# Kotomiya07/kuzushiji-vision

Hardware: AMD Instinct MI355X
Metric: line-images/sec (train) (higher is better)
Workload: dtype bf16; 1 GPU; TrOCR train step: ViT-B/16 (12L/768/12h/3072) on 64x640 crops (S_e=161) + RoBERTa decoder 6L/256/4h/768, V=4300 one-char vocab, labels [B,128], dropout 0.1, clip 1.0, RAdamScheduleFree; BASELINE.json configs[1]; per_gpu_batch=256, global_batch=256, parallelism=dp1

## Files before the change

include/kzv.h:

```cpp
#ifndef KZV_H
#define KZV_H
#include <stddef.h>
#include <stdint.h>

#ifdef __cplusplus
extern "C" {
#endif

#define KZV_OK 0
#define KZV_E_ARG (-1)
#define KZV_E_HIP (-2)
#define KZV_E_STATE (-3)

const char* kzv_last_error(void);
int kzv_version(void);

typedef struct kzv_config {
    int32_t image_h, image_w, patch_h, patch_w, channels;
    int32_t enc_hidden, enc_layers, enc_heads, enc_ffn;
    int32_t dec_hidden, dec_layers, dec_heads, dec_ffn;
    int32_t vocab, max_pos, type_vocab, pad_id;
    float enc_hidden_dropout, enc_attn_dropout, dec_hidden_dropout, dec_attn_dropout;
    float ln_eps;
} kzv_config;
// ... 89 lines not shown
    const void* B; int64_t ldb;
    void* C; int64_t ldc;
    const float* bias;
    const float* resid; int64_t ldr;
    void* aux; int64_t ldaux;
    int32_t M, N, K, n_valid;
    float drop_p; uint32_t drop_key;
} kzv_gemm_nt_args;
int kzv_gemm_nt(const kzv_gemm_nt_args* a, int epilogue, void* stream);
int kzv_set_rows_max_m(int n);
int kzv_set_nt_schedule(int n);
int kzv_set_nt_half_epilogues(int mask);
int kzv_set_nt_half_stagger(int us);
int kzv_set_tn_schedule(int n);
typedef struct kzv_gemm_rows_ln_args {
    const void* A; int64_t lda;
    const void* B; int64_t ldb;
    void* C; int64_t ldc;
    const float* bias;
    void* aux; int64_t ldaux;
    int32_t M, N, K, n_valid;
    const float* ln_a; const float* ln_a_gamma; const float* ln_a_beta;
    const float* ln_r; const float* ln_r_gamma; const float* ln_r_beta;
    float eps;
} kzv_gemm_rows_ln_args;
int kzv_gemm_rows_ln(const kzv_gemm_rows_ln_args* a, int epilogue, void* stream);

typedef struct kzv_gemm_nt_fp8_args {
    const void* A; int64_t lda;
    const void* B; int64_t ldb;
    const float* a_scale;
    const float* b_scale;
    void* C; int64_t ldc;
    const float* bias;
    const float* resid; int64_t ldr;
    void* aux; int64_t ldaux;
    void* c8; int64_t ldc8;
    const float* c8_qscale; float* c8_amax;
    int32_t M, N, K, n_valid;
    float drop_p; uint32_t drop_key;
    const float* c8_rowq;
} kzv_gemm_nt_fp8_args;
int kzv_gemm_nt_fp8(const kzv_gemm_nt_fp8_args* a, int epilogue, void* stream);
int kzv_quant_rows_fp8(const float* x, int64_t rows, int64_t cols, void* q, float* scale, void* stream);
int kzv_layernorm_fwd_fp8(const float* x, const float* gamma, const float* beta, void* y_bf16, void* y_fp8, float* y_scale,
                          float* stats, int rows, int H, float eps, void* stream);
int kzv_set_fp8(kzv_model* m, int mode);
int kzv_get_fp8(const kzv_model* m);
int kzv_fp8_act_scales(const kzv_model* m, float* d_out, void* stream);

typedef struct kzv_gemm_tn_args {
    const void* P; int64_t ldp;
    const void* Q; int64_t ldq;
    float* OUT; int64_t ldo;
    int32_t Mtok, N, K, n_store;
    float* dbias;
} kzv_gemm_tn_args;
int kzv_gemm_tn(const kzv_gemm_tn_args* a, void* stream);

int kzv_gemm_dgrad_wgrad(const kzv_gemm_nt_args* nt, int epilogue, const kzv_gemm_tn_args* tn, void* stream);
int kzv_set_pair(int on);

int kzv_gemm_nt_f32(const kzv_gemm_nt_args* a, int epilogue, void* stream);
int kzv_gemm_tn_f32(const kzv_gemm_tn_args* a, void* stream);

int kzv_layernorm_fwd(const float* x, const float* gamma, const float* beta, void* y_bf16, float* y_f32,
                      float* stats , int rows, int H, float eps, void* stream);
int kzv_layernorm_bwd(const void* dy, int dy_is_f32, const float* x, const float* stats, const float* gamma,
                      float* dx, int accumulate_dx, float* dgamma, float* dbeta, int rows, int H, void* stream);

typedef struct kzv_attn_args {
    const void* Q; const void* K; const void* V;
    void* O;
    float* LSE;
    const void* dO; void* dQ; void* dK; void* dV;
    int64_t ldq, ldk, ldv, ldo;
    const int64_t* ids; int64_t ld_ids; int32_t pad_id;
    int32_t B, heads, Sq, Sk, mode;
    float drop_p; uint32_t drop_key;
    int32_t head_dim;
} kzv_attn_args;
int kzv_attn_fwd(const kzv_attn_args* a, void* stream);
int kzv_attn_bwd(const kzv_attn_args* a, void* stream);
#define KZV_ATTN_MFMA64 1
#define KZV_ATTN_MFMA96 2
#define KZV_ATTN_VALU 3
int kzv_attn_impl(const kzv_attn_args* a, int bwd);

int kzv_attn_stream_fwd(const kzv_attn_args* a, void* stream);
int kzv_attn_stream_bwd(const kzv_attn_args* a, void* stream);
#define KZV_ATTN_STREAM64 4
#define KZV_ATTN_STREAM96 5
int kzv_attn_impl_ex(const kzv_attn_args* a, int bwd, unsigned flags);

int kzv_ocr_set_precision(int fp32);
int kzv_ocr_nchw_to_nhwc(const float* x, void* out_bf16, int N, int C, int H, int W, void* stream);
int kzv_ocr_im2col(const void* x_bf16, void* cols_bf16, int N, int H, int W, int C, int KH, int KW, int stride, int pad, int Kp, void* stream);
int kzv_ocr_col2im(const float* dcols, float* dx, int N, int H, int W, int C, int KH, int KW, int stride, int pad, int Kp, int accumulate, void* stream);
int kzv_ocr_conv_weight(const float* w, void* wp_bf16, void* wpT_bf16, int Cout, int Cin, int KH, int KW, int Kp, void* stream);
int kzv_ocr_conv_wgrad_unpack(const float* gp, float* g, int Cout, int Cin, int KH, int KW, int Kp, void* stream);
int kzv_ocr_conv_weight_multi(int n, const float* const* w, void* const* wp_bf16, void* const* wpT_bf16, const int32_t* geom, void* stream);
int kzv_ocr_conv_wgrad_unpack_multi(int n, const float* const* gp, float* const* g, const int32_t* geom, void* stream);
int64_t kzv_ocr_bn_scratch_floats(int64_t M, int C);
int kzv_ocr_bn_fwd(const float* y, int64_t M, int C, const float* gamma, const float* beta, float* run_mean, float* run_var, float* mean,
                   float* rstd, const void* resid_bf16, void* out_bf16, int relu, int train, float eps, float momentum, float* d_scratch, void* stream);
int kzv_ocr_bn_bwd(const float* da, const void* a_bf16, const float* y, int64_t M, int C, const float* mean, const float* rstd, const float* gamma,
                   float* dz, float* dgamma, float* dbeta, void* dy_bf16, int relu, int train, float* d_scratch, void* stream);
int kzv_ocr_maxpool_fwd(const void* x_bf16, void* out_bf16, unsigned char* idx, int N, int H, int W, int C, void* stream);
int kzv_ocr_maxpool_bwd(const float* dout, const unsigned char* idx, float* dx, int N, int H, int W, int C, void* stream);
int kzv_ocr_avgpool_fwd(const void* x_bf16, float* feat_f32, void* feat_bf16, int N, int HW, int C, void* stream);
int kzv_ocr_avgpool_bwd(const float* dfeat, float* dx, int N, int HW, int C, void* stream);
int kzv_ocr_lstm_cell_fwd(const float* gates, const float* b_hh, float* h_f32, void* h_bf16, int64_t ldh, int B, int H, void* stream);
int kzv_ocr_lstm_cell_bwd(const float* gates, const float* b_hh, const float* dh, int64_t lddh, void* dgates_bf16, int B, int H, void* stream);
int kzv_ocr_log_softmax(const float* x, float* lp, int rows, int C, void* stream);
int kzv_ocr_ctc(const float* lp, const int64_t* targets, int64_t ld_targets, const int64_t* input_lengths, const int64_t* target_lengths, int T,
                int B, int C, int blank, int zero_infinity, int max_target_len, float* d_scratch, float* d_nll, const float* d_gscale,
                float* d_dlogits, void* stream);
int kzv_ocr_smooth_l1_boxes(const float* pred, int max_boxes, const float* gt, int gt_boxes, const int32_t* counts, int B, float* d_loss,
                            float* d_dpred, void* stream);
int kzv_ocr_adam(float* p, const float* g, float* m, float* v, int64_t n, float lr, float beta1, float beta2, float eps, int step, void* stream);
int kzv_ocr_adam_dev(float* p, const float* g, float* m, float* v, int64_t n, float lr, float beta1, float beta2, float eps, const float* d_bc,
                     void* stream);
int kzv_ocr_cast_bf16(const float* x, void* out_bf16, int64_t n, void* stream);
int kzv_ocr_cast_transpose(const float* x, void* out_bf16, int rows, int cols, void* stream);

int kzv_prof_enable(int on, int capacity);
int kzv_prof_select(unsigned kind_mask);
int kzv_prof_collect(int kind, double* total_ms, double* total_flops, int64_t* launches);
int kzv_prof_sample(int stride);
int64_t kzv_prof_seen(int kind);
uint32_t kzv_drop_key(uint64_t seed, uint32_t site);

#define KZV_SITE_ENC_EMB 1u
#define KZV_SITE_ENC_LAYER(i, k) (16u + 4u * (uint32_t)(i) + (uint32_t)(k))
#define KZV_SITE_DEC_EMB 1000u
#define KZV_SITE_DEC_LAYER(i, k) (1016u + 8u * (uint32_t)(i) + (uint32_t)(k))

int kzv_debug_dropout_mask(uint32_t key, float p, int64_t rows, int64_t cols, int64_t ld_index, float* d_out, void* stream);
int kzv_debug_attn_dropout_mask(uint32_t key, float p, int64_t pairs, int32_t Sq, int32_t Sk, float* d_out, void* stream);

int kzv_set_cu_reserve(int n);
int kzv_get_cu_reserve(void);

typedef struct {
    int64_t src_off;
    int64_t tmp_off;
    int64_t hb_off, hk_off;
    int64_t vb_off, vk_off;
    int32_t in_h, in_w, new_h, new_w, paste_x, paste_y, hk_size, vk_size;
} kzv_line_desc;
int kzv_lanczos_coeffs(int in_size, int out_size, int32_t* bounds, int32_t* kk, int* ksize);
int kzv_preprocess_lines(const uint8_t* rgb, const kzv_line_desc* desc, const int32_t* coef, int n, int target_h, int target_w,
                         int64_t max_tmp_pixels, const float* lut256, uint8_t* tmp, float* out, void* stream);

#ifdef __cplusplus
}
#endif
#endif
```

kuzushiji-vision_amd/csrc/attention.hip:

```cpp
#define KZV_GLDS_NT
#include "attention_common.h"

namespace {


struct AttnP {
    const bf16_t* Q; const bf16_t* K; const bf16_t* V; bf16_t* O; float* LSE;
    const bf16_t* dO; bf16_t* dQ; bf16_t* dK; bf16_t* dV;
    const void* zero16;
    int64_t ldq, ldk, ldv, ldo;
    const int64_t* ids; int64_t ld_ids; int pad_id;
    int B, heads, Sq, Sk;
    float scale; unsigned thr16; float inv_keep; unsigned key;
};

template <int SP, int NW>
__device__ __forceinline__ void stage_image(char* img, const bf16_t* src, int64_t ld, int nvalid, const void* zero16,
                                            int w, int lane) {
    const int r8 = lane >> 3;
    for (int pc = w; pc < SP / 8; pc += NW) {
        const int row = pc * 8 + r8;
        const int chunk = (lane & 7) ^ swz<64>(row);
        const void* s = row < nvalid ? (const void*)(src + (int64_t)row * ld + chunk * 8) : zero16;
        glds16(s, img + pc * 1024);
    }
}

template <int MODE, int NKT, bool EXACT>
__global__ __launch_bounds__(256, NKT <= 12 ? 3 : 2) void attn_fwd_kernel(const AttnP p) {
    constexpr int NKP = (NKT + 1) / 2;
    constexpr int SPK = NKT * 16, SPV = NKP * 32;
    constexpr int QI = (NKT + 3) / 4;
    extern __shared__ __attribute__((aligned(16))) char smem[];
    char* Ks = smem; char* Vs = smem + SPK * 128;
    int* kvalid = (int*)(smem + (SPK + SPV) * 128);
    const int tid = threadIdx.x, lane = tid & 63, w = tid >> 6, g = lane >> 4, l15 = lane & 15;
    const int b = blockIdx.x / p.heads, h = blockIdx.x - b * p.heads;
#ifdef KZV_STAMPS
    unsigned long long* stp = (p.dQ && (blockIdx.x % 257) == 0 && tid == 0) ? (unsigned long long*)p.dQ + (blockIdx.x / 257) * 8 : nullptr;
    int stk = 0;
#define KZV_ASTAMP() do { if (stp) stp[stk++] = __builtin_amdgcn_s_memrealtime(); } while (0)
#else
#define KZV_ASTAMP() do {} while (0)
#endif
    KZV_ASTAMP();
    stage_image<SPK, 4>(Ks, p.K + (int64_t)b * p.Sk * p.ldk + h * 64, p.ldk, p.Sk, p.zero16, w, lane);
    stage_image<SPV, 4>(Vs, p.V + (int64_t)b * p.Sk * p.ldv + h * 64, p.ldv, p.Sk, p.zero16, w, lane);
    if (MODE == 1)
        for (int i = tid; i < SPK; i += 256) kvalid[i] = i < p.Sk && p.ids[(int64_t)b * p.ld_ids + i] != p.pad_id;
    const int nkt = EXACT ? NKT : (p.Sk + 15) >> 4, nqt = (p.Sq + 15) >> 4;
    bf16x8 qf[QI][2];
#pragma unroll
    for (int it = 0; it < QI; ++it) {
        const int qc = min((w + 4 * it) * 16 + l15, p.Sq - 1);
        const bf16_t* qrow = p.Q + ((int64_t)b * p.Sq + qc) * p.ldq + h * 64 + 8 * g;
        qf[it][0] = *(const bf16x8*)qrow; qf[it][1] = *(const bf16x8*)(qrow + 32);
    }
    const unsigned kA = l15 * 128 + ((g ^ (l15 & 7)) << 4), kB = l15 * 128 + (((4 + g) ^ (l15 & 7)) << 4);
    unsigned vT[4];
    {
        const int row = 4 * g + (l15 >> 2), hb = (l15 >> 1) & 1;
#pragma unroll
        for (int dt = 0; dt < 4; ++dt) vT[dt] = row * 128 + ((((dt * 2 + hb) ^ (row & 7))) << 4) + (l15 & 1) * 8;
    }
    const AttDropLane dl = att_drop_lane(l15 & 3, true);
    const unsigned thrm1x2 = att_thrm1x2(p.thr16);
    const unsigned nQ4 = KZV_ATT_N4(p.Sq), nK4 = KZV_ATT_N4(p.Sk);
    asm volatile("s_waitcnt vmcnt(0)" ::: "memory");
    __syncthreads();
    KZV_ASTAMP();

    const float sc = p.scale * LOG2E;
#pragma unroll
    for (int it = 0; it < QI; ++it) {
        const int qt = w + 4 * it;
        if (qt >= nqt) break;
        const int q = qt * 16 + l15;
        const bf16x8 q0 = qf[it][0], q1 = qf[it][1];
        const int nk = MODE == 1 ? min(nkt, qt + 1) : nkt;
        f32x4 s[NKT];
        float mx = -INFINITY;
#pragma unroll
        for (int kt = 0; kt < NKT; ++kt) {
            s[kt] = (f32x4){0.f, 0.f, 0.f, 0.f};
            if (EXACT || kt < nk) {
                s[kt] = __builtin_amdgcn_mfma_f32_16x16x32_bf16(*(const bf16x8*)(Ks + kA + kt * 2048), q0, s[kt], 0, 0, 0);
                s[kt] = __builtin_amdgcn_mfma_f32_16x16x32_bf16(*(const bf16x8*)(Ks + kB + kt * 2048), q1, s[kt], 0, 0, 0);
                if (MODE == 1 || (EXACT ? kt == NKT - 1 : kt >= nkt - 1)) {
#pragma unroll
                    for (int r = 0; r < 4; ++r) {
                        const int key = kt * 16 + 4 * g + r;
                        const bool ok = MODE == 0 ? key < p.Sk : (kvalid[key] && key <= q);
                        s[kt][r] = ok ? s[kt][r] : -INFINITY;
                    }
                }
                mx = fmax3(mx, fmax3(s[kt][0], s[kt][1], s[kt][2]), s[kt][3]);
            }
        }
        mx = fmaxf(mx, __shfl_xor(mx, 16, 64));
        mx = fmaxf(mx, __shfl_xor(mx, 32, 64));
        const bool dead = mx == -INFINITY;
        const float mref = dead ? 0.f : mx * sc;
        float sum = 0.f;
        unsigned pw[NKP * 4];
        const unsigned xw0 = att_block_word(b * p.heads + h, nQ4, (unsigned)q >> 2, nK4, g, p.key);
#pragma unroll
        for (int kt = 0; kt < NKP * 2; ++kt) {
            if (kt < NKT && (EXACT || kt < nk)) {
                att_fwd_tile(s[kt], sc, mref, sum, p.thr16, dl, xw0 + (unsigned)kt * (4u * KZV_ATT_GOLD), thrm1x2, pw + kt * 2);
            } else {
                pw[kt * 2] = 0u; pw[kt * 2 + 1] = 0u;
            }
        }
        sum += __shfl_xor(sum, 16, 64);
        sum += __shfl_xor(sum, 32, 64);
        if (p.LSE && g == 0 && q < p.Sq)
            p.LSE[((int64_t)b * p.heads + h) * p.Sq + q] = dead ? INFINITY : (mx * sc + log2f(sum)) * (1.f / LOG2E);
        f32x4 o[4];
#pragma unroll
        for (int dt = 0; dt < 4; ++dt) o[dt] = (f32x4){0.f, 0.f, 0.f, 0.f};
#pragma unroll
        for (int kp = 0; kp < NKP; ++kp) {
            if (EXACT || 2 * kp < nk) {
                const bf16x8 pf = words8(pw[kp * 4], pw[kp * 4 + 1], pw[kp * 4 + 2], pw[kp * 4 + 3]);
#pragma unroll
                for (int dt = 0; dt < 4; ++dt) {
                    const bf16x8 vf = cat8(lds_tr16(Vs + vT[dt] + kp * 4096), lds_tr16(Vs + vT[dt] + kp * 4096 + 2048));
                    o[dt] = __builtin_amdgcn_mfma_f32_16x16x32_bf16(vf, pf, o[dt], 0, 0, 0);
                }
            }
        }
        const float onorm = dead ? 0.f : p.inv_keep / sum;
        if (q < p.Sq) {
            bf16_t* orow = p.O + ((int64_t)b * p.Sq + q) * p.ldo + h * 64 + 4 * g;
#pragma unroll
            for (int dt = 0; dt < 4; ++dt)
                store_bf4(orow + dt * 16, o[dt], onorm);
        }
        KZV_ASTAMP();
    }
}

constexpr int SLAB = 32 * 128;
constexpr bool bwd_ds(int MODE, int NKT, int NW, bool EXACT) { return NW == 4 && (EXACT || (MODE == 1 && NKT <= 8)); }
constexpr int bwd_lds_bytes(int NKT, int MODE, bool DS) {
    return ((NKT + 1) / 2 * 32) * 128 + NKT * 16 * 128 + 4 * SLAB + ((NKT + 1) / 2 * 32) * 64 + (MODE == 1 ? 3 : 2) * ((NKT + 1) / 2 * 32) * 4 + (DS ? SLAB : 0);
}
static_assert(bwd_lds_bytes(11, 0, true) <= 80 * 1024 && bwd_lds_bytes(12, 0, false) <= 80 * 1024 && bwd_lds_bytes(8, 1, true) <= 80 * 1024,
              "attention backward (<= 192 tokens) must fit two workgroups per CU");

template <int NW>
__device__ __forceinline__ void stage_slabs(char* qs, char* os, const bf16_t* Qb, const bf16_t* dOb, unsigned ldq, unsigned ldo,
                                            int row0, int nvalid, int w, int lane, char* oo = nullptr, const bf16_t* Ob = nullptr) {
    const int npc = oo ? 12 : 8;
    for (int pc = w; pc < npc; pc += NW) {
        const int pq = pc & 3;
        const int row = pq * 8 + (lane >> 3);
        const unsigned chunk = (lane & 7) ^ swz<64>(row);
        const unsigned r = (unsigned)min(row0 + row, nvalid - 1);
        if (pc < 4) glds16_asm_soff_m0(Qb, (r * ldq + chunk * 8) * 2, qs + pq * 1024);
        else if (pc < 8) glds16_asm_soff_m0(dOb, (r * ldo + chunk * 8) * 2, os + pq * 1024);
        else glds16_asm_soff_m0(Ob, (r * ldo + chunk * 8) * 2, oo + pq * 1024);
    }
}
__device__ __forceinline__ void slab_delta(const char* os, const char* oo, float* dlt_slab, float keep_p, int w, int lane) {
    const int row = w * 8 + (lane >> 3);
    const unsigned off = img_off<64>(row, lane & 7);
    const bf16x8 a = *(const bf16x8*)(os + off), e = *(const bf16x8*)(oo + off);
    float d = dot8(a, e);
    d += __shfl_xor(d, 1, 64);
    d += __shfl_xor(d, 2, 64);
    d += __shfl_xor(d, 4, 64);
    if ((lane & 7) == 0) dlt_slab[row] = d * keep_p;
}
template <int SP, int NW>
__device__ __forceinline__ void stage_image_asm(char* img, const bf16_t* src, int64_t ld, int nvalid, const void* zero16,
                                                int w, int lane) {
    const int r8 = lane >> 3;
    for (int pc = w; pc < SP / 8; pc += NW) {
        const int row = pc * 8 + r8;
        const int chunk = (lane & 7) ^ swz<64>(row);
        glds16_asm_m0(row < nvalid ? (const void*)(src + (int64_t)row * ld + chunk * 8) : zero16, img + pc * 1024);
    }
}

#ifdef KZV_STAMPS
__device__ unsigned long long kzv_bwd_stamps[128];
#define KZV_BSTAMP() do { if (blockIdx.x == 771 && threadIdx.x == 0 && bsk < 128) kzv_bwd_stamps[bsk++] = __builtin_amdgcn_s_memrealtime(); } while (0)
#else
#define KZV_BSTAMP() do {} while (0)
#endif
template <int MODE, int NKT, int NW, bool EXACT>
__global__ __launch_bounds__(NW * 64, 2) void attn_bwd_kernel(const AttnP p) {
    [[maybe_unused]] int bsk = 0;
    KZV_BSTAMP();
    constexpr int NKP = (NKT + 1) / 2, SP = NKP * 32;
    constexpr int NT = NW * 64, TPW = (NKT + NW - 1) / NW, TB = 8 / NW;
    static_assert(TPW <= 3, "dK/dV accumulators of more than 3 key tiles per wave do not fit the register file");
    extern __shared__ __attribute__((aligned(16))) char smem[];
    char* Ks = smem; char* Vs = Ks + SP * 128;
    char* Qring = Vs + NKT * 16 * 128; char* Oring = Qring + 2 * SLAB;
    char* dST = Oring + 2 * SLAB;
    constexpr bool DS = bwd_ds(MODE, NKT, NW, EXACT);
    float* lse = (float*)(dST + SP * 64);
    float* dlt = lse + SP;
    char* Oo = (char*)(dlt + SP);
    int* kvalid = (int*)(Oo + (DS ? SLAB : 0));
    const int tid = threadIdx.x, lane = tid & 63, w = tid >> 6, g = lane >> 4, l15 = lane & 15;
    const int b = blockIdx.x / p.heads, h = blockIdx.x - b * p.heads;
    const bf16_t* Qb = p.Q + (int64_t)b * p.Sq * p.ldq + h * 64;
    const bf16_t* dOb = p.dO + (int64_t)b * p.Sq * p.ldo + h * 64;
    const bf16_t* Ob = p.O + (int64_t)b * p.Sq * p.ldo + h * 64;
    const float keep_p = 1.f / p.inv_keep;
  if constexpr (DS) {
    float lv = INFINITY;
    if (tid < SP && tid < p.Sq) lv = p.LSE[((int64_t)b * p.heads + h) * p.Sq + tid] * LOG2E;
    stage_slabs<NW>(Qring, Oring, Qb, dOb, (unsigned)p.ldq, (unsigned)p.ldo, 0, p.Sq, w, lane, Oo, Ob);
    stage_image_asm<SP, NW>(Ks, p.K + (int64_t)b * p.Sk * p.ldk + h * 64, p.ldk, p.Sk, p.zero16, w, lane);
    stage_image_asm<NKT * 16, NW>(Vs, p.V + (int64_t)b * p.Sk * p.ldv + h * 64, p.ldv, p.Sk, p.zero16, w, lane);
    KZV_BSTAMP();
    if (tid < SP) lse[tid] = lv;
    for (int row = tid; row < SP; row += NT) if (row >= 32) dlt[row] = 0.f;
    KZV_BSTAMP();
  } else {
    constexpr int DR = (SP + NT / 4 - 1) / (NT / 4);
    bf16x8 ov[DR][2], dv8[DR][2];
    float lv[DR];
#pragma unroll
    for (int i = 0; i < DR; ++i) {
        const int row = min((tid >> 2) + i * (NT / 4), p.Sq - 1);
        const bf16_t* orow = p.O + ((int64_t)b * p.Sq + row) * p.ldo + h * 64 + (tid & 3) * 16;
        const bf16_t* drow = dOb + (int64_t)row * p.ldo + (tid & 3) * 16;
        ov[i][0] = *(const bf16x8*)orow; ov[i][1] = *(const bf16x8*)(orow + 8);
        dv8[i][0] = *(const bf16x8*)drow; dv8[i][1] = *(const bf16x8*)(drow + 8);
        lv[i] = p.LSE[((int64_t)b * p.heads + h) * p.Sq + row];
    }
    stage_image_asm<SP, NW>(Ks, p.K + (int64_t)b * p.Sk * p.ldk + h * 64, p.ldk, p.Sk, p.zero16, w, lane);
    stage_image_asm<NKT * 16, NW>(Vs, p.V + (int64_t)b * p.Sk * p.ldv + h * 64, p.ldv, p.Sk, p.zero16, w, lane);
    stage_slabs<NW>(Qring, Oring, Qb, dOb, (unsigned)p.ldq, (unsigned)p.ldo, 0, p.Sq, w, lane);
    KZV_BSTAMP();
#pragma unroll
    for (int i = 0; i < DR; ++i) {
        const int row = (tid >> 2) + i * (NT / 4);
        float d = 0.f;
#pragma unroll
        for (int c = 0; c < 2; ++c) d = dot8(ov[i][c], dv8[i][c], d);
        att_row_stats(d, lv[i], keep_p, row, SP, p.Sq, tid, lse, dlt);
    }
    KZV_BSTAMP();
  }
    if (MODE == 1)
        for (int row = tid; row < SP; row += NT) kvalid[row] = row < p.Sk && p.ids[(int64_t)b * p.ld_ids + row] != p.pad_id;
    for (int i = tid; i < SP * 64 / 16; i += NT) ((uint4*)dST)[i] = make_uint4(0, 0, 0, 0);
    asm volatile("s_waitcnt vmcnt(0)" ::: "memory");
    if constexpr (DS) slab_delta(Oring, Oo, dlt, keep_p, w, lane);
    __syncthreads();
    KZV_BSTAMP();

    const int nkt = EXACT ? NKT : (p.Sk + 15) >> 4, nqb = (p.Sq + 31) >> 5;
    const float sc = p.scale * LOG2E;
    f32x4 dk[TPW][4], dv[TPW][4];
#pragma unroll
    for (int a = 0; a < TPW; ++a)
#pragma unroll
        for (int d = 0; d < 4; ++d) { dk[a][d] = (f32x4){0.f, 0.f, 0.f, 0.f}; dv[a][d] = (f32x4){0.f, 0.f, 0.f, 0.f}; }
    const unsigned rA = img_off<64>(l15, g), rB = img_off<64>(l15, 4 + g);
    unsigned tT[4];
    {
        const int row = 4 * g + (l15 >> 2), hb = (l15 >> 1) & 1;
#pragma unroll
        for (int dt = 0; dt < 4; ++dt) tT[dt] = row * 128 + ((((dt * 2 + hb) ^ (row & 7))) << 4) + (l15 & 1) * 8;
    }
    const AttDropLane dl = att_drop_lane(l15 & 3, false);
    const int thr_s = att_thr_s(p.thr16);
    const unsigned nQ4 = KZV_ATT_N4(p.Sq), nK4 = KZV_ATT_N4(p.Sk);
    unsigned xslab = att_block_word(b * p.heads + h, nQ4, g, nK4, l15 >> 2, p.key);
    const unsigned xstep_t2 = 4u * nK4 * KZV_ATT_GOLD;

    for (int qb = 0; qb < nqb; ++qb) {
        const char* Qs = Qring + (qb & 1) * SLAB;
        const char* Os = Oring + (qb & 1) * SLAB;
        bf16x8 Qr[2][2], Or[2][2];
#pragma unroll
        for (int t2 = 0; t2 < 2; ++t2) {
            Qr[t2][0] = *(const bf16x8*)(Qs + rA + t2 * 2048); Qr[t2][1] = *(const bf16x8*)(Qs + rB + t2 * 2048);
            Or[t2][0] = *(const bf16x8*)(Os + rA + t2 * 2048); Or[t2][1] = *(const bf16x8*)(Os + rB + t2 * 2048);
        }
        if (qb + 1 < nqb)
            stage_slabs<NW>(Qring + ((qb + 1) & 1) * SLAB, Oring + ((qb + 1) & 1) * SLAB, Qb, dOb, (unsigned)p.ldq, (unsigned)p.ldo, (qb + 1) * 32, p.Sq, w, lane,
                            DS ? Oo : nullptr, Ob);
        KZV_BSTAMP();
#pragma unroll
        for (int a = 0; a < TPW; ++a) {
            const int kt = w + NW * a;
            if (kt >= nkt) continue;
            const int key = kt * 16 + l15;
            char* dsrow = dST + key * 64;
            const int dsz = (key >> 1) & 7;
            if (MODE == 1 && kt * 16 > qb * 32 + 31) {
#pragma unroll
                for (int t2 = 0; t2 < 2; ++t2) *(uint2*)(dsrow + (((t2 * 4 + g) ^ dsz) << 3)) = make_uint2(0u, 0u);
                continue;
            }
            const bf16x8 k0 = *(const bf16x8*)(Ks + rA + kt * 2048), k1 = *(const bf16x8*)(Ks + rB + kt * 2048);
            const bf16x8 v0 = *(const bf16x8*)(Vs + rA + kt * 2048), v1 = *(const bf16x8*)(Vs + rB + kt * 2048);
            const bool kok = MODE == 1 ? kvalid[key] != 0 : key < p.Sk;
            const float sinit = kok ? 0.f : -INFINITY;
            unsigned pdw[4], dsw[4];
#pragma unroll
            for (int t2 = 0; t2 < 2; ++t2) {
                const f32x4 lq4 = *(const f32x4*)(lse + qb * 32 + t2 * 16 + 4 * g), dq4 = *(const f32x4*)(dlt + qb * 32 + t2 * 16 + 4 * g);
                f32x4 S = (f32x4){sinit, sinit, sinit, sinit}, dP = (f32x4){0.f, 0.f, 0.f, 0.f};
                S = __builtin_amdgcn_mfma_f32_16x16x32_bf16(Qr[t2][0], k0, S, 0, 0, 0);
                S = __builtin_amdgcn_mfma_f32_16x16x32_bf16(Qr[t2][1], k1, S, 0, 0, 0);
                dP = __builtin_amdgcn_mfma_f32_16x16x32_bf16(Or[t2][0], v0, dP, 0, 0, 0);
                dP = __builtin_amdgcn_mfma_f32_16x16x32_bf16(Or[t2][1], v1, dP, 0, 0, 0);
                unsigned u01 = 0, u23 = 0;
                if (p.thr16)
                    att_drop_u(dl, att_mix(xslab + (unsigned)t2 * xstep_t2 + (unsigned)kt * (4u * KZV_ATT_GOLD)), &u01, &u23);
                float pm[4], ds[4];
#pragma unroll
                for (int r = 0; r < 4; ++r)
                    att_bwd_elem<MODE == 1>(r, S[r], dP[r], sc, lq4[r], dq4[r], key <= qb * 32 + t2 * 16 + 4 * g + r, u01, u23, thr_s, pm[r], ds[r]);
                pdw[t2 * 2] = pack_bf2(pm[0], pm[1]); pdw[t2 * 2 + 1] = pack_bf2(pm[2], pm[3]);
                dsw[t2 * 2] = pack_bf2(ds[0], ds[1]); dsw[t2 * 2 + 1] = pack_bf2(ds[2], ds[3]);
                *(uint2*)(dsrow + (((t2 * 4 + g) ^ dsz) << 3)) = make_uint2(dsw[t2 * 2], dsw[t2 * 2 + 1]);
            }
            const bf16x8 pf = words8(pdw[0], pdw[1], pdw[2], pdw[3]), df = words8(dsw[0], dsw[1], dsw[2], dsw[3]);
#pragma unroll
            for (int dt = 0; dt < 4; ++dt) {
                const bf16x8 dOt = cat8(lds_tr16(Os + tT[dt]), lds_tr16(Os + tT[dt] + 2048));
                const bf16x8 Qt = cat8(lds_tr16(Qs + tT[dt]), lds_tr16(Qs + tT[dt] + 2048));
                dv[a][dt] = __builtin_amdgcn_mfma_f32_16x16x32_bf16(dOt, pf, dv[a][dt], 0, 0, 0);
                dk[a][dt] = __builtin_amdgcn_mfma_f32_16x16x32_bf16(Qt, df, dk[a][dt], 0, 0, 0);
            }
            KZV_BSTAMP();
        }
        KZV_BSTAMP();
        __syncthreads();
        KZV_BSTAMP();
        {
            const int t2 = w / (NW / 2), dt0 = (w % (NW / 2)) * TB;
            const int q = qb * 32 + t2 * 16 + l15;
            f32x4 acc[TB];
#pragma unroll
            for (int u = 0; u < TB; ++u) acc[u] = (f32x4){0.f, 0.f, 0.f, 0.f};
            const int krow = 8 * g + (l15 >> 2);
            const unsigned dA = krow * 64 + (((t2 * 4 + (l15 & 3)) ^ ((krow >> 1) & 7)) << 3);
            const unsigned dB = (krow + 4) * 64 + (((t2 * 4 + (l15 & 3)) ^ (((krow + 4) >> 1) & 7)) << 3);
            unsigned kT[TB][2];
#pragma unroll
            for (int u = 0; u < TB; ++u) {
                const int row = 8 * g + (l15 >> 2), chunk = (dt0 + u) * 2 + ((l15 >> 1) & 1);
                kT[u][0] = row * 128 + ((chunk ^ (row & 7)) << 4) + (l15 & 1) * 8;
                kT[u][1] = (row + 4) * 128 + ((chunk ^ ((row + 4) & 7)) << 4) + (l15 & 1) * 8;
            }
            const int nks = EXACT ? NKP : (nkt + 1) >> 1;
#pragma unroll
            for (int ks = 0; ks < NKP; ++ks) {
                if (EXACT || ks < nks) {
                    const bf16x8 dsf = cat8(lds_tr16(dST + dA + ks * 2048), lds_tr16(dST + dB + ks * 2048));
#pragma unroll
                    for (int u = 0; u < TB; ++u) {
                        const bf16x8 kf = cat8(lds_tr16(Ks + kT[u][0] + ks * 4096), lds_tr16(Ks + kT[u][1] + ks * 4096));
                        acc[u] = __builtin_amdgcn_mfma_f32_16x16x32_bf16(kf, dsf, acc[u], 0, 0, 0);
                    }
                }
            }
            KZV_BSTAMP();
            asm volatile("s_waitcnt vmcnt(0)" ::: "memory");
            if constexpr (DS)
                if (qb + 1 < nqb) slab_delta(Oring + ((qb + 1) & 1) * SLAB, Oo, dlt + (qb + 1) * 32, keep_p, w, lane);
            if (q < p.Sq) {
                const float osc = p.scale * p.inv_keep;
                bf16_t* row = p.dQ + ((int64_t)b * p.Sq + q) * p.ldq + h * 64 + 4 * g;
#pragma unroll
                for (int u = 0; u < TB; ++u) {
                    const int dt = dt0 + u;
                    *(uint2*)(row + dt * 16) = make_uint2(pack_bf2(acc[u][0] * osc, acc[u][1] * osc), pack_bf2(acc[u][2] * osc, acc[u][3] * osc));
                }
            }
        }
        xslab += 2u * xstep_t2;
        KZV_BSTAMP();
        __syncthreads();
        KZV_BSTAMP();
    }
    const float ksc = p.scale * p.inv_keep;
#pragma unroll
    for (int a = 0; a < TPW; ++a) {
        const int key = (w + NW * a) * 16 + l15;
        if (w + NW * a >= nkt || key >= p.Sk) continue;
        bf16_t* krow = p.dK + ((int64_t)b * p.Sk + key) * p.ldk + h * 64 + 4 * g;
        bf16_t* vrow = p.dV + ((int64_t)b * p.Sk + key) * p.ldv + h * 64 + 4 * g;
#pragma unroll
        for (int dt = 0; dt < 4; ++dt) {
            store_bf4(krow + dt * 16, dk[a][dt], ksc);
            store_bf4(vrow + dt * 16, dv[a][dt], p.inv_keep);
        }
    }
}

}

#ifdef KZV_STAMPS
extern "C" int kzv_debug_bwd_stamps(unsigned long long* host128) {
    return hipMemcpyFromSymbol(host128, HIP_SYMBOL(kzv_bwd_stamps), 128 * sizeof(unsigned long long)) == hipSuccess ? 0 : 1;
}
#endif

template <int MODE, int NKT, bool EXACT>
static void launch_fwd(const AttnP& p, int blocks, hipStream_t s) {
    constexpr int lds = (NKT * 16 + (NKT + 1) / 2 * 32) * 128 + NKT * 16 * 4;
    static bool attr = false;
    if (!attr) { (void)hipFuncSetAttribute((const void*)attn_fwd_kernel<MODE, NKT, EXACT>, hipFuncAttributeMaxDynamicSharedMemorySize, lds); attr = true; }
    hipLaunchKernelGGL((attn_fwd_kernel<MODE, NKT, EXACT>), dim3(blocks), dim3(256), lds, s, p);
}
template <int MODE, int NKT, int NW, bool EXACT>
static void launch_bwd(const AttnP& p, int blocks, hipStream_t s) {
    constexpr int lds = bwd_lds_bytes(NKT, MODE, bwd_ds(MODE, NKT, NW, EXACT));
    static bool attr = false;
    if (!attr) { (void)hipFuncSetAttribute((const void*)attn_bwd_kernel<MODE, NKT, NW, EXACT>, hipFuncAttributeMaxDynamicSharedMemorySize, lds); attr = true; }
    hipLaunchKernelGGL((attn_bwd_kernel<MODE, NKT, NW, EXACT>), dim3(blocks), dim3(NW * 64), lds, s, p);
}

int kzv_attn_mfma64(const kzv_attn_args* a, bool bwd, hipStream_t s) {
    AttnP p;
    kzv_attn_fill(p, a, 64);
    if (int rc = kzv_attn_fill_zero(p, "attn")) return rc;
    p.ids = a->ids; p.ld_ids = a->ld_ids; p.pad_id = a->pad_id;
    const int nkt = (a->Sk + 15) >> 4, nqt = (a->Sq + 15) >> 4, nqb = (a->Sq + 31) >> 5, blocks = a->B * a->heads;
    if (!bwd) {
        if (a->mode == 1) launch_fwd<1, 12, false>(p, blocks, s);
        else if (nkt == 11 && nqt <= 12) launch_fwd<0, 11, true>(p, blocks, s);
        else if (nkt == 10 && nqt <= 12) launch_fwd<0, 10, true>(p, blocks, s);
        else if (nkt <= 12 && nqt <= 12) launch_fwd<0, 12, false>(p, blocks, s);
        else launch_fwd<0, 18, false>(p, blocks, s);
        return kzv_check_launch("attn_fwd");
    }
    if (a->mode == 1 && nkt <= 8) launch_bwd<1, 8, 4, false>(p, blocks, s);
    else if (a->mode == 1) launch_bwd<1, 12, 4, false>(p, blocks, s);
    else if (nkt == 11 && nqb <= 6) launch_bwd<0, 11, 4, true>(p, blocks, s);
    else if (nkt == 10 && nqb <= 5) launch_bwd<0, 10, 4, true>(p, blocks, s);
    else if (nkt <= 12 && nqb <= 6) launch_bwd<0, 12, 4, false>(p, blocks, s);
    else launch_bwd<0, 18, 8, false>(p, blocks, s);
    return kzv_check_launch("attn_bwd");
}
```

kuzushiji-vision_amd/kzv/_lib.py:

```python
from __future__ import annotations

import ctypes as C
import os

_HERE = os.path.dirname(os.path.abspath(__file__))
LIB_PATH = os.environ.get("KZV_LIB") or os.path.join(_HERE, "libkzv.so")


class KzvError(RuntimeError):
    pass


class kzv_config(C.Structure):
    _fields_ = [(n, C.c_int32) for n in (
        "image_h", "image_w", "patch_h", "patch_w", "channels",
        "enc_hidden", "enc_layers", "enc_heads", "enc_ffn",
        "dec_hidden", "dec_layers", "dec_heads", "dec_ffn",
        "vocab", "max_pos", "type_vocab", "pad_id")] + [(n, C.c_float) for n in (
        "enc_hidden_dropout", "enc_attn_dropout", "dec_hidden_dropout", "dec_attn_dropout", "ln_eps")]


class kzv_opt_step(C.Structure):
    _fields_ = [("lr_t", C.c_float), ("ckp1", C.c_float), ("beta1", C.c_float), ("beta2", C.c_float),
                ("eps", C.c_float), ("weight_decay", C.c_float), ("bias_correction2", C.c_float),
# ... 28 lines not shown

class kzv_beam_state(C.Structure):
    _fields_ = [("batch", C.c_int32), ("num_beams", C.c_int32), ("max_len", C.c_int32), ("vocab", C.c_int32), ("eos_id", C.c_int32),
                ("run_seq_in", C.c_void_p), ("run_seq_out", C.c_void_p), ("fin_seq_in", C.c_void_p), ("fin_seq_out", C.c_void_p),
                ("run_scores", C.c_void_p), ("fin_scores", C.c_void_p), ("fin_done", C.c_void_p), ("fin_len", C.c_void_p),
                ("unsatisfied", C.c_void_p)]


class kzv_gemm_tn_args(C.Structure):
    _fields_ = [("P", C.c_void_p), ("ldp", C.c_int64), ("Q", C.c_void_p), ("ldq", C.c_int64),
                ("OUT", C.c_void_p), ("ldo", C.c_int64),
                ("Mtok", C.c_int32), ("N", C.c_int32), ("K", C.c_int32), ("n_store", C.c_int32),
                ("dbias", C.c_void_p)]


class kzv_attn_args(C.Structure):
    _fields_ = [("Q", C.c_void_p), ("K", C.c_void_p), ("V", C.c_void_p), ("O", C.c_void_p), ("LSE", C.c_void_p),
                ("dO", C.c_void_p), ("dQ", C.c_void_p), ("dK", C.c_void_p), ("dV", C.c_void_p),
                ("ldq", C.c_int64), ("ldk", C.c_int64), ("ldv", C.c_int64), ("ldo", C.c_int64),
                ("ids", C.c_void_p), ("ld_ids", C.c_int64), ("pad_id", C.c_int32),
                ("B", C.c_int32), ("heads", C.c_int32), ("Sq", C.c_int32), ("Sk", C.c_int32), ("mode", C.c_int32),
                ("drop_p", C.c_float), ("drop_key", C.c_uint32), ("head_dim", C.c_int32)]


EPI_BF16, EPI_F32, EPI_GELU, EPI_RESID, EPI_DGELU = range(5)
ATTN_MFMA64, ATTN_MFMA96, ATTN_VALU = 1, 2, 3
ATTN_STREAM64, ATTN_STREAM96 = 4, 5
ATTN_IMPL_NAMES = {ATTN_MFMA64: "mfma64", ATTN_MFMA96: "mfma96", ATTN_VALU: "valu", ATTN_STREAM64: "stream64", ATTN_STREAM96: "stream96"}
MODEL_LONG_SEQ = 1

_P = C.c_void_p
class kzv_line_desc(C.Structure):
    _fields_ = [("src_off", C.c_int64), ("tmp_off", C.c_int64), ("hb_off", C.c_int64), ("hk_off", C.c_int64),
                ("vb_off", C.c_int64), ("vk_off", C.c_int64), ("in_h", C.c_int32), ("in_w", C.c_int32), ("new_h", C.c_int32),
                ("new_w", C.c_int32), ("paste_x", C.c_int32), ("paste_y", C.c_int32), ("hk_size", C.c_int32), ("vk_size", C.c_int32)]


SYMBOLS = {
    "kzv_last_error": (C.c_char_p, []),
    "kzv_version": (C.c_int, []),
    "kzv_model_create": (C.c_int, [C.POINTER(kzv_config), C.POINTER(_P)]),
    "kzv_model_create_ex": (C.c_int, [C.POINTER(kzv_config), C.c_uint, C.POINTER(_P)]),
    "kzv_model_destroy": (C.c_int, [_P]),
    "kzv_param_count": (C.c_int, [_P]),
    "kzv_param_info": (C.c_int, [_P, C.c_int, C.POINTER(C.c_char_p), C.POINTER(C.c_int64),
                                 C.POINTER(C.c_int64), C.POINTER(C.c_int64)]),
    "kzv_param_total": (C.c_int64, [_P]),
    "kzv_workspace_bytes": (C.c_int64, [_P, C.c_int, C.c_int]),
    "kzv_model_bind": (C.c_int, [_P, _P, _P, _P, C.c_int64, C.c_int, C.c_int]),
    "kzv_model_sync_weights": (C.c_int, [_P, _P]),
    "kzv_forward_loss": (C.c_int, [_P, _P, _P, _P, _P, C.c_int, C.c_uint64, _P]),
    "kzv_set_image_width": (C.c_int, [_P, C.c_int]),
    "kzv_check_positions": (C.c_int, [_P, _P]),
    "kzv_encode_images": (C.c_int, [_P, _P, C.c_int, _P]),
    "kzv_set_active_length": (C.c_int, [_P, C.c_int]),
    "kzv_decode_logits": (C.c_int, [_P, _P, C.c_int, _P, _P]),
    "kzv_zero_grads": (C.c_int, [_P, _P]),
    "kzv_backward_segments": (C.c_int, [_P]),
    "kzv_backward_segment": (C.c_int, [_P, C.c_int, _P]),
    "kzv_backward_segment_range": (C.c_int, [_P, C.c_int, C.POINTER(C.c_int64), C.POINTER(C.c_int64)]),
    "kzv_backward": (C.c_int, [_P, _P]),
    "kzv_grad_sqnorm": (C.c_int, [_P, C.c_int64, _P, _P, _P]),
    "kzv_clip_and_step": (C.c_int, [_P, _P, _P, _P, C.c_int64, _P, C.POINTER(kzv_opt_step), _P]),
    "kzv_clip_and_step_ema": (C.c_int, [_P, _P, _P, _P, C.c_int64, _P, C.POINTER(kzv_opt_step), _P, C.c_float, _P]),
    "kzv_lerp_params": (C.c_int, [_P, _P, C.c_int64, C.c_float, _P]),
    "kzv_gemm_nt": (C.c_int, [C.POINTER(kzv_gemm_nt_args), C.c_int, _P]),
    "kzv_set_rows_max_m": (C.c_int, [C.c_int]),
    "kzv_set_nt_schedule": (C.c_int, [C.c_int]),
    "kzv_set_nt_half_epilogues": (C.c_int, [C.c_int]),
    "kzv_set_nt_half_stagger": (C.c_int, [C.c_int]),
    "kzv_set_tn_schedule": (C.c_int, [C.c_int]),
    "kzv_gemm_rows_ln": (C.c_int, [C.POINTER(kzv_gemm_rows_ln_args), C.c_int, _P]),
    "kzv_gemm_nt_fp8": (C.c_int, [C.POINTER(kzv_gemm_nt_fp8_args), C.c_int, _P]),
    "kzv_quant_rows_fp8": (C.c_int, [_P, C.c_int64, C.c_int64, _P, _P, _P]),
    "kzv_layernorm_fwd_fp8": (C.c_int, [_P, _P, _P, _P, _P, _P, _P, C.c_int, C.c_int, C.c_float, _P]),
    "kzv_set_fp8": (C.c_int, [_P, C.c_int]),
    "kzv_get_fp8": (C.c_int, [_P]),
    "kzv_fp8_act_scales": (C.c_int, [_P, _P, _P]),
    "kzv_gemm_tn": (C.c_int, [C.POINTER(kzv_gemm_tn_args), _P]),
    "kzv_layernorm_fwd": (C.c_int, [_P, _P, _P, _P, _P, _P, C.c_int, C.c_int, C.c_float, _P]),
    "kzv_layernorm_bwd": (C.c_int, [_P, C.c_int, _P, _P, _P, _P, C.c_int, _P, _P, C.c_int, C.c_int, _P]),
    "kzv_attn_fwd": (C.c_int, [C.POINTER(kzv_attn_args), _P]),
    "kzv_attn_bwd": (C.c_int, [C.POINTER(kzv_attn_args), _P]),
    "kzv_attn_impl": (C.c_int, [C.POINTER(kzv_attn_args), C.c_int]),
    "kzv_attn_stream_fwd": (C.c_int, [C.POINTER(kzv_attn_args), _P]),
    "kzv_attn_stream_bwd": (C.c_int, [C.POINTER(kzv_attn_args), _P]),
    "kzv_attn_impl_ex": (C.c_int, [C.POINTER(kzv_attn_args), C.c_int, C.c_uint]),
    "kzv_drop_key": (C.c_uint32, [C.c_uint64, C.c_uint32]),
    "kzv_debug_dropout_mask": (C.c_int, [C.c_uint32, C.c_float, C.c_int64, C.c_int64, C.c_int64, _P, _P]),
    "kzv_debug_attn_dropout_mask": (C.c_int, [C.c_uint32, C.c_float, C.c_int64, C.c_int32, C.c_int32, _P, _P]),
    "kzv_gemm_dgrad_wgrad": (C.c_int, [C.POINTER(kzv_gemm_nt_args), C.c_int, C.POINTER(kzv_gemm_tn_args), _P]),
    "kzv_set_pair": (C.c_int, [C.c_int]),
    "kzv_gemm_nt_f32": (C.c_int, [C.POINTER(kzv_gemm_nt_args), C.c_int, _P]),
    "kzv_gemm_tn_f32": (C.c_int, [C.POINTER(kzv_gemm_tn_args), _P]),
    "kzv_ocr_set_precision": (C.c_int, [C.c_int]),
    "kzv_ocr_nchw_to_nhwc": (C.c_int, [_P, _P, C.c_int, C.c_int, C.c_int, C.c_int, _P]),
    "kzv_ocr_im2col": (C.c_int, [_P, _P] + [C.c_int] * 9 + [_P]),
    "kzv_ocr_col2im": (C.c_int, [_P, _P] + [C.c_int] * 10 + [_P]),
    "kzv_ocr_conv_weight": (C.c_int, [_P, _P, _P] + [C.c_int] * 5 + [_P]),
    "kzv_ocr_conv_wgrad_unpack": (C.c_int, [_P, _P] + [C.c_int] * 5 + [_P]),
    "kzv_ocr_conv_weight_multi": (C.c_int, [C.c_int, _P, _P, _P, _P, _P]),
    "kzv_ocr_conv_wgrad_unpack_multi": (C.c_int, [C.c_int, _P, _P, _P, _P]),
    "kzv_ocr_bn_fwd": (C.c_int, [_P, C.c_int64, C.c_int, _P, _P, _P, _P, _P, _P, _P, _P, C.c_int, C.c_int, C.c_float, C.c_float, _P, _P]),
    "kzv_ocr_bn_bwd": (C.c_int, [_P, _P, _P, C.c_int64, C.c_int, _P, _P, _P, _P, _P, _P, _P, C.c_int, C.c_int, _P, _P]),
    "kzv_ocr_bn_scratch_floats": (C.c_int64, [C.c_int64, C.c_int]),
    "kzv_ocr_maxpool_fwd": (C.c_int, [_P, _P, _P, C.c_int, C.c_int, C.c_int, C.c_int, _P]),
    "kzv_ocr_maxpool_bwd": (C.c_int, [_P, _P, _P, C.c_int, C.c_int, C.c_int, C.c_int, _P]),
    "kzv_ocr_avgpool_fwd": (C.c_int, [_P, _P, _P, C.c_int, C.c_int, C.c_int, _P]),
    "kzv_ocr_avgpool_bwd": (C.c_int, [_P, _P, C.c_int, C.c_int, C.c_int, _P]),
    "kzv_ocr_lstm_cell_fwd": (C.c_int, [_P, _P, _P, _P, C.c_int64, C.c_int, C.c_int, _P]),
    "kzv_ocr_lstm_cell_bwd": (C.c_int, [_P, _P, _P, C.c_int64, _P, C.c_int, C.c_int, _P]),
    "kzv_ocr_log_softmax": (C.c_int, [_P, _P, C.c_int, C.c_int, _P]),
    "kzv_ocr_ctc": (C.c_int, [_P, _P, C.c_int64, _P, _P, C.c_int, C.c_int, C.c_int, C.c_int, C.c_int, C.c_int, _P, _P, _P, _P, _P]),
    "kzv_ocr_smooth_l1_boxes": (C.c_int, [_P, C.c_int, _P, C.c_int, _P, C.c_int, _P, _P, _P]),
    "kzv_ocr_adam": (C.c_int, [_P, _P, _P, _P, C.c_int64, C.c_float, C.c_float, C.c_float, C.c_float, C.c_int, _P]),
    "kzv_ocr_adam_dev": (C.c_int, [_P, _P, _P, _P, C.c_int64, C.c_float, C.c_float, C.c_float, C.c_float, _P, _P]),
    "kzv_ocr_cast_bf16": (C.c_int, [_P, _P, C.c_int64, _P]),
    "kzv_ocr_cast_transpose": (C.c_int, [_P, _P, C.c_int, C.c_int, _P]),
    "kzv_prof_enable": (C.c_int, [C.c_int, C.c_int]),
    "kzv_prof_select": (C.c_int, [C.c_uint]),
    "kzv_prof_sample": (C.c_int, [C.c_int]),
    "kzv_prof_seen": (C.c_int64, [C.c_int]),
    "kzv_set_cu_reserve": (C.c_int, [C.c_int]),
    "kzv_get_cu_reserve": (C.c_int, []),
    "kzv_decode_step": (C.c_int, [C.c_void_p, C.c_void_p, C.c_void_p, C.c_int, C.c_void_p, C.c_int64, C.c_void_p, C.c_void_p]),
    "kzv_decode_begin": (C.c_int, [C.c_void_p, C.c_void_p]),
    "kzv_set_decode_one_launch": (C.c_int, [C.c_int]),
    "kzv_set_dec_chain": (C.c_int, [C.c_int]),
    "kzv_set_head_ce": (C.c_int, [C.c_int]),
    "kzv_decode_step_graph": (C.c_int, [C.c_void_p, C.c_void_p, C.c_void_p, C.c_void_p, C.c_int64, C.c_void_p, C.c_void_p]),
    "kzv_decode_reorder": (C.c_int, [C.c_void_p, C.c_void_p, C.c_int, C.c_void_p]),
    "kzv_decode_prep": (C.c_int, [C.c_void_p, C.c_int64, C.c_int, C.c_int, C.c_int, C.c_void_p, C.c_void_p, C.c_int64, C.c_void_p, C.c_void_p]),
    "kzv_greedy_update": (C.c_int, [C.c_void_p, C.c_int64, C.c_int, C.c_void_p, C.c_int64, C.c_int, C.c_void_p, C.c_int, C.c_int, C.c_int,
                                    C.c_void_p, C.c_void_p]),
    "kzv_beam_update": (C.c_int, [C.POINTER(kzv_beam_state), C.c_void_p, C.c_void_p, C.c_int, C.c_int, C.c_float, C.c_void_p, C.c_void_p, C.c_void_p]),
    "kzv_beam_topk": (C.c_int, [C.c_void_p, C.c_int64, C.c_void_p, C.c_int, C.c_int, C.c_int, C.c_int, C.c_void_p, C.c_void_p, C.c_void_p]),
    "kzv_lanczos_coeffs": (C.c_int, [C.c_int, C.c_int, C.c_void_p, C.c_void_p, C.POINTER(C.c_int)]),
    "kzv_preprocess_lines": (C.c_int, [C.c_void_p, C.c_void_p, C.c_void_p, C.c_int, C.c_int, C.c_int, C.c_int64, C.c_void_p,
                                       C.c_void_p, C.c_void_p, C.c_void_p]),
    "kzv_prof_collect": (C.c_int, [C.c_int, C.POINTER(C.c_double), C.POINTER(C.c_double), C.POINTER(C.c_int64)]),
}

_lib = None


def load() -> C.CDLL:
    global _lib
    if _lib is not None:
        return _lib
    if not os.path.exists(LIB_PATH):
        raise KzvError(f"{LIB_PATH} not built -- run `python -c 'import __graft_entry__ as g; g.build()'` "
                       "(hipcc --offload-arch=gfx950).  There is no CPU fallback.")
    import torch
    lib = C.CDLL(LIB_PATH)
    for name, (res, args) in SYMBOLS.items():
        fn = getattr(lib, name)
        fn.restype = res
        fn.argtypes = args
    _lib = lib
    return lib


def check(rc: int, what: str = "") -> None:
    if rc != 0:
        msg = load().kzv_last_error().decode("utf-8", "replace")
        raise KzvError(f"{what or 'libkzv'} failed ({rc}): {msg}")
# ... 30 lines not shown
```

Measured before the change: 8396 img/s.

## Prefetch next wave's attention head K/V/Q into cache during compute

```diff
diff --git a/include/kzv.h b/include/kzv.h
--- a/include/kzv.h
+++ b/include/kzv.h
@@ -195,6 +195,7 @@
 } kzv_attn_args;
 int kzv_attn_fwd(const kzv_attn_args* a, void* stream);
 int kzv_attn_bwd(const kzv_attn_args* a, void* stream);
+int kzv_set_attn_prefetch(int on);
 #define KZV_ATTN_MFMA64 1
 #define KZV_ATTN_MFMA96 2
 #define KZV_ATTN_VALU 3
diff --git a/kuzushiji-vision_amd/csrc/attention.hip b/kuzushiji-vision_amd/csrc/attention.hip
--- a/kuzushiji-vision_amd/csrc/attention.hip
+++ b/kuzushiji-vision_amd/csrc/attention.hip
@@ -12,6 +12,7 @@
     const int64_t* ids; int64_t ld_ids; int pad_id;
     int B, heads, Sq, Sk;
     float scale; unsigned thr16; float inv_keep; unsigned key;
+    unsigned pf;
 };
 
 template <int SP, int NW>
@@ -26,11 +27,44 @@
     }
 }
 
+struct PfSlot { const char* base; unsigned r0, mul, n, stride; };
+__device__ __forceinline__ PfSlot pf_rows(const bf16_t* op, int64_t ld, int b, int h, int S, int n, int i) {
+    return {(const char*)(op + (int64_t)b * S * ld + h * 64), (unsigned)i * 64u, 1u, (unsigned)n, (unsigned)ld * 2u};
+}
+__device__ __forceinline__ unsigned pf_off(const PfSlot& s, unsigned lane) { return min(s.r0 + lane * s.mul, s.n - 1u) * s.stride; }
+__device__ __forceinline__ void pf_retire(unsigned sink) { asm volatile("; prefetch sink %0 retired" : : "v"(sink)); }
+
+template <bool BWD>
+__device__ __forceinline__ void pf_next_head(int w, int lane, unsigned& sink) {
+    typedef const __attribute__((address_space(4))) AttnP KernargP;
+    KernargP* kp = (KernargP*)__builtin_amdgcn_kernarg_segment_ptr();
+    unsigned ln = lane;
+    asm volatile("" : "+s"(kp), "+v"(ln));
+    KernargP& p = *kp;
+    const int nb = blockIdx.x + p.pf;
+    const int b = nb / p.heads, h = nb - b * p.heads;
+    const int ws = __builtin_amdgcn_readfirstlane(w);
+    const int nkc = (p.Sk + 63) >> 6, nqc = BWD ? 4 : (p.Sq + 63) >> 6;
+#pragma unroll 1
+    for (int c = ws; c < 2 * nkc + nqc; c += 4) {
+        PfSlot s;
+        if (c < nkc) s = pf_rows(p.K, p.ldk, b, h, p.Sk, p.Sk, c);
+        else if (c < 2 * nkc) s = pf_rows(p.V, p.ldv, b, h, p.Sk, p.Sk, c - nkc);
+        else if (!BWD) s = pf_rows(p.Q, p.ldq, b, h, p.Sq, p.Sq, c - 2 * nkc);
+        else if (c == 2 * nkc) s = pf_rows(p.Q, p.ldq, b, h, p.Sq, min(p.Sq, 32), 0);
+        else if (c == 2 * nkc + 1) s = pf_rows(p.dO, p.ldo, b, h, p.Sq, min(p.Sq, 32), 0);
+        else if (c == 2 * nkc + 2) s = pf_rows(p.O, p.ldo, b, h, p.Sq, min(p.Sq, 32), 0);
+        else s = {(const char*)(p.LSE + ((int64_t)b * p.heads + h) * p.Sq), 0u, 32u, (unsigned)p.Sq, 4u};
+        asm volatile("global_load_dword %0, %1, %2" : "+v"(sink) : "v"(pf_off(s, ln)), "s"(s.base));
+    }
+}
+
 template <int MODE, int NKT, bool EXACT>
 __global__ __launch_bounds__(256, NKT <= 12 ? 3 : 2) void attn_fwd_kernel(const AttnP p) {
     constexpr int NKP = (NKT + 1) / 2;
     constexpr int SPK = NKT * 16, SPV = NKP * 32;
     constexpr int QI = (NKT + 3) / 4;
+    constexpr bool PF = MODE == 0 && NKT <= 12;
     extern __shared__ __attribute__((aligned(16))) char smem[];
     char* Ks = smem; char* Vs = smem + SPK * 128;
     int* kvalid = (int*)(smem + (SPK + SPV) * 128);
@@ -63,9 +97,10 @@
 #pragma unroll
         for (int dt = 0; dt < 4; ++dt) vT[dt] = row * 128 + ((((dt * 2 + hb) ^ (row & 7))) << 4) + (l15 & 1) * 8;
     }
-    const AttDropLane dl = att_drop_lane(l15 & 3, true);
+    AttDropLane dl = att_drop_lane(l15 & 3, true);
     const unsigned thrm1x2 = att_thrm1x2(p.thr16);
     const unsigned nQ4 = KZV_ATT_N4(p.Sq), nK4 = KZV_ATT_N4(p.Sk);
+    if constexpr (PF) pin(dl);
     asm volatile("s_waitcnt vmcnt(0)" ::: "memory");
     __syncthreads();
     KZV_ASTAMP();
@@ -75,6 +110,8 @@
     for (int it = 0; it < QI; ++it) {
         const int qt = w + 4 * it;
         if (qt >= nqt) break;
+        [[maybe_unused]] unsigned pfsink = 0;
+        if constexpr (PF) if (it == 0 && blockIdx.x + p.pf < gridDim.x) pf_next_head<false>(w, lane, pfsink);
         const int q = qt * 16 + l15;
         const bf16x8 q0 = qf[it][0], q1 = qf[it][1];
         const int nk = MODE == 1 ? min(nkt, qt + 1) : nkt;
@@ -131,6 +168,8 @@
             }
         }
         const float onorm = dead ? 0.f : p.inv_keep / sum;
+        if constexpr (PF)
+            if (it == 0) { asm volatile("s_waitcnt vmcnt(0)"); pf_retire(pfsink); }
         if (q < p.Sq) {
             bf16_t* orow = p.O + ((int64_t)b * p.Sq + q) * p.ldo + h * 64 + 4 * g;
 #pragma unroll
@@ -289,6 +328,9 @@
         if (qb + 1 < nqb)
             stage_slabs<NW>(Qring + ((qb + 1) & 1) * SLAB, Oring + ((qb + 1) & 1) * SLAB, Qb, dOb, (unsigned)p.ldq, (unsigned)p.ldo, (qb + 1) * 32, p.Sq, w, lane,
                             DS ? Oo : nullptr, Ob);
+        [[maybe_unused]] unsigned pfsink = 0;
+        const bool pfetch = DS && qb == (nqb > 1) && blockIdx.x + p.pf < gridDim.x;
+        if constexpr (DS) if (pfetch) pf_next_head<true>(w, lane, pfsink);
         KZV_BSTAMP();
 #pragma unroll
         for (int a = 0; a < TPW; ++a) {
@@ -369,6 +411,7 @@
             }
             KZV_BSTAMP();
             asm volatile("s_waitcnt vmcnt(0)" ::: "memory");
+            if constexpr (DS) if (pfetch) pf_retire(pfsink);
             if constexpr (DS)
                 if (qb + 1 < nqb) slab_delta(Oring + ((qb + 1) & 1) * SLAB, Oo, dlt + (qb + 1) * 32, keep_p, w, lane);
             if (q < p.Sq) {
@@ -424,12 +467,29 @@
     hipLaunchKernelGGL((attn_bwd_kernel<MODE, NKT, NW, EXACT>), dim3(blocks), dim3(NW * 64), lds, s, p);
 }
 
+static int g_attn_prefetch = -1;
+static bool attn_prefetch() {
+    if (g_attn_prefetch < 0) { const char* e = getenv("KZV_ATTN_PREFETCH"); g_attn_prefetch = e ? (atoi(e) != 0) : 1; }
+    return g_attn_prefetch != 0;
+}
+extern "C" int kzv_set_attn_prefetch(int on) { g_attn_prefetch = on < 0 ? -1 : (on != 0); return KZV_OK; }
+static unsigned attn_pf_distance(int per_cu) {
+    static int cus = 0;
+    if (!cus) {
+        int dev = 0, n = 0;
+        if (hipGetDevice(&dev) != hipSuccess || hipDeviceGetAttribute(&n, hipDeviceAttributeMultiprocessorCount, dev) != hipSuccess || n <= 0) n = 256;
+        cus = n;
+    }
+    return attn_prefetch() ? (unsigned)(cus * per_cu + 7) & ~7u : 1u << 30;
+}
+
 int kzv_attn_mfma64(const kzv_attn_args* a, bool bwd, hipStream_t s) {
     AttnP p;
     kzv_attn_fill(p, a, 64);
     if (int rc = kzv_attn_fill_zero(p, "attn")) return rc;
     p.ids = a->ids; p.ld_ids = a->ld_ids; p.pad_id = a->pad_id;
     const int nkt = (a->Sk + 15) >> 4, nqt = (a->Sq + 15) >> 4, nqb = (a->Sq + 31) >> 5, blocks = a->B * a->heads;
+    p.pf = attn_pf_distance(bwd ? 2 : 3);
     if (!bwd) {
         if (a->mode == 1) launch_fwd<1, 12, false>(p, blocks, s);
         else if (nkt == 11 && nqt <= 12) launch_fwd<0, 11, true>(p, blocks, s);
diff --git a/kuzushiji-vision_amd/kzv/_lib.py b/kuzushiji-vision_amd/kzv/_lib.py
--- a/kuzushiji-vision_amd/kzv/_lib.py
+++ b/kuzushiji-vision_amd/kzv/_lib.py
@@ -134,6 +134,7 @@
     "kzv_layernorm_bwd": (C.c_int, [_P, C.c_int, _P, _P, _P, _P, C.c_int, _P, _P, C.c_int, C.c_int, _P]),
     "kzv_attn_fwd": (C.c_int, [C.POINTER(kzv_attn_args), _P]),
     "kzv_attn_bwd": (C.c_int, [C.POINTER(kzv_attn_args), _P]),
+    "kzv_set_attn_prefetch": (C.c_int, [C.c_int]),
     "kzv_attn_impl": (C.c_int, [C.POINTER(kzv_attn_args), C.c_int]),
     "kzv_attn_stream_fwd": (C.c_int, [C.POINTER(kzv_attn_args), _P]),
     "kzv_attn_stream_bwd": (C.c_int, [C.POINTER(kzv_attn_args), _P]),
```

After: 8339 img/s. Within noise of the previous version (-0.7%).
